# scottschroeder/shirley-raytracing-rs

Measured on AMD Instinct MI355X. Metric: Msamples/sec (whole node) on book-1 random_scene 1200x800 @ 500spp; 1/2/4/8 GPU, higher is better.
Workload: dtype f64

## Files before the change

### shirley-raytracing-rs_amd/csrc/rt/rt_api.cpp

```cpp
#include <algorithm>
#include <cmath>
#include <cstdlib>
#include <cstring>
#include <limits>
#include <string>
#include <vector>

#include "adaptive.h"
#include "plan.h"
#include "rt_ctx.h"

using namespace rt;

namespace rt {

int ensure(rt_ctx* c, DevBuf& b, size_t bytes) {
  if (b.bytes >= bytes && b.p) return RT_OK;
  if (c) HIP_TRY(c, hipSetDevice(c->device));
  if (b.p) {
    (void)hipFree(b.p);
    b.p = nullptr;
    b.bytes = 0;
  }
  if (bytes == 0) return RT_OK;
// ... 362 lines not shown
      w.q_window = (uint32_t)std::max(1, atoi(e) / kWave) * (uint32_t)kWave;
    KBlock& kb = c->host_blocks[k];
    kb.cam = kp.cam;
    kb.scene = kp.scene;
    kb.work = w;
    kb.partial = kp.partial;
    kb.unit_counter = kp.unit_counter;
    kb.counters = kp.counters;
    kb.ground = c->place.hop_kind == 2 ? static_cast<const DGround*>(c->ground.p) : nullptr;
    void* kdev = static_cast<KBlock*>(c->kcam.p) + k;
    HIP_TRY(c, hipMemcpyAsync(kdev, &kb, sizeof(KBlock), hipMemcpyHostToDevice, s));
    kp.kconst = (uint64_t)(uintptr_t)kdev;
    HIP_TRY(c, hipMemsetAsync(c->unit_counter.p, 0, std::max<size_t>(64, (size_t)nseg * sizeof(uint32_t)), s));
    HIP_TRY(c, hipEventRecord(c->pass_ev[2 * k], s));
    if (engine == RT_ENGINE_WAVEFRONT) {
      st = run_wavefront(c, kp, timing, s);
      if (st) return st;
    } else if (engine == RT_ENGINE_SPLIT) {
      kp.split_refill = c->split_refill;
      KParams ks = kp;
      ks.scene.n_lds_mats = ks.scene.n_lds_texs = 0;
      HIP_TRY(c, launch_split(ks, c->split_nt, c->cu_count, s));
    } else {
      HIP_TRY(c, launch_trace(kp, (int)nseg, c->place.mk_threads, c->place.hop_kind, s));
    }
    HIP_TRY(c, hipEventRecord(c->pass_ev[2 * k + 1], s));
    if (k == passes - 1) HIP_TRY(c, hipEventRecord(c->ev[1], s));
    if (step)
      HIP_TRY(c, launch_fold_stats(kp.partial, w.n_chunks, step->n_list, step->list_dev, L.tiles_x, cam->image_width,
                                   cam->image_height, step->batches_before + c1, step->batch, step->noise_floor,
                                   out_dev, step->moments_dev, step->err_dev, s));
    else
      HIP_TRY(c, launch_reduce(kp.partial, w.n_chunks, L.n_tiles_rank, L.tiles_x, ty0, p->tile_rank, p->tile_world,
                               cam->image_width, row0, row1, packed, k > 0 ? 1 : 0, out_dev, s));
    c->last_passes = k + 1;
  }
  HIP_TRY(c, hipEventRecord(c->ev[2], s));
  c->have_timing = true;
  return RT_OK;
}

}

extern "C" {

const char* rt_version(void) { return "shirley-rt 0.2 (gfx950, f64 wavefront + persistent megakernel)"; }

// ... 89 lines not shown
  if ((st = up(c->prim_light, cs.prim_light))) return st;
  if ((st = ensure(c, c->shutter0, 2 * sizeof(double)))) return st;
  HIP_TRY(c, hipMemset(c->shutter0.p, 0, 2 * sizeof(double)));

  DScene& S = c->scene;
  S.nodes = static_cast<const DNode*>(c->nodes.p);
  S.nodes4 = c->nodes4.p;
  S.prims = static_cast<const DPrim*>(c->prims.p);
  S.mats = static_cast<const DMat*>(c->mats.p);
  S.texs = static_cast<const DTex*>(c->texs.p);
  S.perlin = static_cast<const DPerlin*>(c->perlin.p);
  S.exts = cs.exts.empty() ? nullptr : static_cast<const DExt*>(c->exts.p);
  S.time0 = S.time1 = 0.0;
  S.shutter = static_cast<const double*>(c->shutter0.p);
  S.n_nodes = (int32_t)cs.nodes.size();
  S.n_nodes4 = cs.stats.n_nodes4;
  S.n_prims = cs.stats.n_objects;
  place_scene(P, S);
  S.sky = d->sky;
  for (int k = 0; k < 3; ++k) S.sky_color[k] = d->sky_color[k];
  c->place = P;

  int bpc = 0;
  HIP_TRY(c, trace_occupancy(S, P.mk_threads, P.hop_kind, &bpc));
  if (bpc < 1) return fail(c, RT_E_UNSUPPORTED, "trace kernel does not fit on a CU (LDS %lld B)", P.stack_bytes);
  c->blocks_per_cu = bpc;
  DScene W = S;
  W.n_lds_mats = W.n_lds_texs = 0;
  W.n_lds_nodes = P.wf_n_lds_nodes;
  int wbpc = 0;
  HIP_TRY(c, wf_prepare(W, &wbpc));
  if (wbpc < 1) return fail(c, RT_E_UNSUPPORTED, "wavefront extend kernel does not fit on a CU");
  c->wf_scene = W;
  c->wf_blocks_per_cu = wbpc;
  c->wf_wide = false;
  if (P.wf_extend4) {
    int b4 = 0;
    HIP_TRY(c, wf_prepare4(S, &b4));
    if (b4 >= 1) {
      c->wf_wide = true;
      c->wf4_blocks_per_cu = b4;
      c->wf_scene = S;
      c->wf_scene.n_lds_mats = c->wf_scene.n_lds_texs = 0;
    }
  }
  c->split_nt = 0;
  if (P.split_nt) {
// ... 418 lines not shown
```

### shirley-raytracing-rs_amd/csrc/rt/rt_device.h

```cpp
#pragma once

#ifdef RT_PORTABLE_LIBM
#include "portable_libm.h"
#define RT_SIN pl_sin
#define RT_LOG pl_log
#define RT_ACOS pl_acos
#define RT_ATAN2 pl_atan2
#define RT_POW5_LIBM(x) pl_pow5(x)
#else
#define RT_SIN sin
#define RT_LOG log
#define RT_ACOS acos
#define RT_ATAN2 atan2
#define RT_POW5_LIBM(x) pow(x, 5.0)
#endif
#include <hip/hip_runtime.h>

#include "../../../include/shirley_rt.h"
#include "rt_layout.h"

namespace rt {


struct v3 {
// ... 812 lines not shown
    } else if (h0) {
      next = c0;
    } else if (h1) {
      next = c1;
    } else {
      next = -1;
      while (sp > 0) {
        --sp;
        if ((double)stk_t[sp * STRIDE] <= t_best) {
          next = stk_node[sp * STRIDE];
          break;
        }
      }
      if (next < 0) break;
    }
    node = next;
  }
  resolve_ties<EXT>(S, o, d, t_min, t_best, best, face_best, rk, seed);
  return best;
}

#ifdef RT_PHASE_TIMING
#define g_trav_lane_steps trav_lane_steps_ref
static __device__ unsigned long long g_phase_ctr[64];
static __device__ unsigned long long g_visit_hist[64], g_wave_visit_hist[64];

__device__ __forceinline__ void ph_count(int i) {
  const unsigned long long act = __ballot(1);
  if ((int)__lane_id() == __builtin_ctzll(act)) {
    atomicAdd(&g_phase_ctr[2 * i], (unsigned long long)__popcll(act));
    atomicAdd(&g_phase_ctr[2 * i + 1], 1ull);
  }
}
#ifndef RT_PHASE_NO_EVENTS
#define PH_COUNT(i) ph_count(i)
#else
#define PH_COUNT(i)
#endif
#else
#define PH_COUNT(i)
#endif
#ifdef RT_PHASE_TIMING
#define RT_STAT(x) x
#define RT_STAT_ARG(x) , x
#else
#define RT_STAT(x)
#define RT_STAT_ARG(x)
// ... 407 lines not shown
__device__ __noinline__ RootHit traverse4_root_ool(const DNode4F* lds_nodes, const DPrim* lds_prims, const DPrim* prims_v,
                                                   int root4, unsigned key_mask, float origin_limit, v3 o, v3 d, Rng rk,
                                                   uint64_t seed_v) {
  DScene S{};
  S.prims = uniform_ptr(prims_v);
  S.root4 = __builtin_amdgcn_readfirstlane(root4);
  S.key_mask = (unsigned)__builtin_amdgcn_readfirstlane((int)key_mask);
  S.origin_limit = __int_as_float(__builtin_amdgcn_readfirstlane(__float_as_int(origin_limit)));
  RootHit r{0, -1, -1, __builtin_inf()};
  unsigned visits = 0, ptests = 0;
  r.ok = traverse4_root<MODE>(S, lds_nodes, lds_prims, o, d, 0.001, r.t, r.best, r.face, rk, uniform64(seed_v), visits,
                              ptests)
             ? 1
             : 0;
  return r;
}
#endif

__device__ __forceinline__ bool box_inward(int face, v3 d) {
  const double da = face < 2 ? d.z : (face < 4 ? d.x : d.y);
  return (face & 1) ? da > 0.0 : da < 0.0;
}
typedef __attribute__((address_space(4))) const DGround GGround;
__device__ __forceinline__ bool ground_hop(const DScene& S, const DPrim* lds_prims, const DMat* mats, GGround* g, v3 o, v3 d,
                                           double t_min, double& t_best, int& best, int& face_best, bool& guarded) {
  bool div_ok;
  const v3 inv = inv_dir(d, div_ok);
  const RaySigns ns = ray_signs(inv);
  t_best = __builtin_inf();
  best = -1;
  face_best = -1;
  const int n = g->n, n_box = g->n_box;
#pragma unroll 1
  for (int i = 0; i < n; ++i) {
    const int leaf = g->prim[i];
    const DPrim& pr = lds_prims[leaf];
    double te, t;
    if (i < n_box) {
      double tx;
      if (!slab_s(pr.p, o, inv, ns, t_min, t_best, te, tx)) {
        mark_tie<false>(best, near_entry(te, t_best));
        continue;
      }
      const int f = div_ok ? box_t1f(pr.p, o, d, inv, ns, t_min, t_best, te, tx, t) : box_t(pr.p, o, d, t_min, t_best, t, inv, div_ok);
      if (f >= 0 && tie_takes<false>(S, leaf, best, t, t_best, o, inv, ns, t_min)) { t_best = t; best = leaf; face_best = f; }
    } else {
      double b[6];
      leaf_box(pr, b);
      if (!slab_s(b, o, inv, ns, t_min, t_best, te)) continue;
      if (rect_t<0, 2>(pr.p, o, d, t_min, t_best, t, inv, div_ok) && tie_takes<false>(S, leaf, best, t, t_best, o, inv, ns, t_min)) {
        t_best = t; best = leaf; face_best = -1;
      }
    }
  }
  guarded = false;
  if (best < 0 || (best & kTieBit) || face_best < 4 || !(t_best > t_min)) return false;
  const DPrim& pb = lds_prims[best];
  const double ay = fabs(d.y);
  bool ok = mats[pb.material].kind == RT_MAT_DIELECTRIC && o.y >= g->y_lo && o.y <= g->y_hi && ay >= g->dy_min &&
            ay <= 0x1p300 && d.x * d.x + d.z * d.z <= g->ratio2 * (d.y * d.y);
  if (ok && (face_best == 4 ? pb.p[4] : pb.p[1]) == g->y_top) {
    const int nx = g->nx;
    const int ix = ground_cell(o.x + t_best * d.x, g->x0, nx), iz = ground_cell(o.z + t_best * d.z, g->z0, g->nz);
    if (ix >= 0 && iz >= 0) {
      typedef __attribute__((address_space(1))) const uint32_t GBits;
      const unsigned c = (unsigned)iz * (unsigned)nx + (unsigned)ix;
      GBits* bits = (GBits*)(uintptr_t)((uint64_t)(uintptr_t)g + sizeof(DGround));
      guarded = (bits[c >> 5] >> (c & 31u)) & 1u;
      ok = !guarded;
    }
  }
  return ok;
}

struct Trav4 {
  v3 inv;
  Recip ra;
  bool ra_ok;
  double t_best;
  float tmaxf;
  int best, face, node, sp, steps;
  unsigned top;
  RaySigns ns;
  RayF rf;
};

template <bool EXT>
__device__ __forceinline__ void trav4_begin(Trav4& T, const DScene& S, v3 o, v3 d, double t_max) {
  bool inv_ok;
  T.inv = inv_dir(d, inv_ok);
  T.ns = ray_signs(T.inv);
  T.rf = ray_f<typename Node4Sel<EXT>::T>(S, o, T.inv);
  T.ra = recip(len2(d));
  T.ra_ok = inv_ok && T.ra.b >= 0x1p-300 && T.ra.b <= 0x1p300 && T.rf.fast;
  T.t_best = t_max;
// ... 767 lines not shown
```

### shirley-raytracing-rs_amd/csrc/rt/rt_layout.h

```cpp
#pragma once

#include <stddef.h>
#include <stdint.h>

#include "plan.h"

namespace rt {

constexpr int kTile = 8;
constexpr int kTilePixels = kTile * kTile;
constexpr int kTraceThreads = 256;
constexpr int kTraceThreadsWide = 1024;
#ifndef RT_EXT_WIDE_THREADS
#define RT_EXT_WIDE_THREADS 768
#endif
constexpr int kTraceThreadsWide3 = RT_EXT_WIDE_THREADS;
constexpr int kHitThreads = 256;
constexpr int kExtendThreads = 256;
constexpr int kWave = 64;
constexpr int kLdsBytes = 160 * 1024;

constexpr int32_t kEmptyChild = 0x7fffffff;
struct alignas(16) DNode {
  double box[2][6];
// ... 114 lines not shown
  int32_t sky;
  double sky_color[3];
  const DExt* exts;
  double time0, time1;
  const double* shutter;
  int32_t n_lds_mats;
  int32_t n_lds_texs;
};

constexpr int kGroundMaxPrims = 4;
constexpr double kGroundCellsPerUnit = 32.0;
constexpr double kGroundCell = 1.0 / kGroundCellsPerUnit;
constexpr double kGroundGuard = 1.0 / 32.0;
constexpr long long kGroundMaxCells = 128LL * 1024 * 8;
struct alignas(16) DGround {
  double y_lo, y_hi;
  double y_top;
  double dy_min;
  double ratio2;
  double x0, z0;
  int32_t nx, nz;
  int32_t n, n_box;
  int32_t prim[kGroundMaxPrims];
  int32_t pad[2];
};
static_assert(sizeof(DGround) == 96, "DGround layout");
#ifdef __HIPCC__
#define RT_HOST_DEVICE __host__ __device__
#else
#define RT_HOST_DEVICE
#endif
RT_HOST_DEVICE inline int ground_cell(double v, double v0, int n) {
  const double q = (v - v0) * kGroundCellsPerUnit;
  return (q >= 0.0 && q < (double)n) ? (int)q : -1;
}

struct DCamera {
  int32_t width, height;
  int32_t has_lens;
  int32_t pad;
  double lens_radius;
  double origin[3], u[3], v[3];
  double horizontal[3], vertical[3], lower_left[3];
  double wd, hd, inv_w, inv_h;
};

struct UDiv {
// ... 117 lines not shown
```

### shirley-raytracing-rs_amd/csrc/rt/scene_compile.cpp

```cpp
#include "scene_compile.h"

#include <algorithm>
#include <cmath>
#include <cstdarg>
#include <cstdio>
#include <cstdlib>
#include <cstring>
#include <limits>

namespace rt {

namespace {
int fail(std::string* err, int code, const char* fmt, ...) {
  char buf[512];
  va_list ap;
  va_start(ap, fmt);
  vsnprintf(buf, sizeof buf, fmt, ap);
  va_end(ap);
  if (err) *err = buf;
  return code;
}
}

SceneTuning tuning_from_env() {
  SceneTuning t;
  if (const char* e = getenv("SHIRLEY_COLLAPSE_DP")) t.collapse_dp = atoi(e) != 0;
  if (const char* e = getenv("SHIRLEY_LDS_NODES")) {
    t.has_lds_nodes = true;
    t.lds_nodes = atoll(e);
  }
  t.no_wide = getenv("SHIRLEY_NO_WIDE") != nullptr;
  t.no_lds_prims = getenv("SHIRLEY_NO_LDS_PRIMS") != nullptr;
  t.no_lds_mats = getenv("SHIRLEY_NO_LDS_MATS") != nullptr;
  t.no_lds_perlin = getenv("SHIRLEY_NO_LDS_PERLIN") != nullptr;
  t.no_hop = getenv("SHIRLEY_NO_HOP") != nullptr;
  if (const char* e = getenv("SHIRLEY_HOP")) t.hop_root = std::strcmp(e, "root") == 0;
  if (const char* e = getenv("SHIRLEY_SAH_BOXW")) t.sah_box_weight = atof(e);
  t.sah_binned = getenv("SHIRLEY_SAH_BINNED") != nullptr;
  t.wf_extend2 = getenv("SHIRLEY_WF_EXTEND2") != nullptr;
  if (const char* e = getenv("SHIRLEY_SPLIT_NT")) t.split_nt = atoi(e);
  if (const char* e = getenv("SHIRLEY_SPLIT_REFILL")) t.split_refill = std::max(1, atoi(e));
  return t;
}

bool is_extended(const rt_object& o) {
  return o.geometry == RT_GEOM_MOVING_SPHERE || o.medium != 0 || o.transform != 0;
}
void rotate_y_cs(const rt_object& o, double& cs, double& sn) {
  const double rad = o.rotate_y_deg * 3.14159265358979323846 / 180.0;
  cs = std::cos(rad);
  sn = std::sin(rad);
}
bool texture_uses_uv(const rt_scene_desc* d, int32_t ti) {
  if (ti < 0 || ti >= d->n_textures) return false;
  const rt_texture& t = d->textures[ti];
  if (t.kind == RT_TEX_IMAGE) return true;
  if (t.kind == RT_TEX_CHECKER) return texture_uses_uv(d, t.odd) || texture_uses_uv(d, t.even);
  return false;
}
// ... 499 lines not shown
    if (!(lo_y >= top) || !(std::fabs(p[0]) <= big && std::fabs(p[1]) <= big && std::fabs(p[2]) <= big)) return false;
    const double dx = std::max(std::fabs(p[0] - ex0), std::fabs(p[0] - ex1));
    const double dy = std::max(std::fabs(p[1] - low), std::fabs(p[1] - top));
    const double dz = std::max(std::fabs(p[2] - ez0), std::fabs(p[2] - ez1));
    dist = std::max(dist, std::sqrt(dx * dx + dy * dy + dz * dz));
    if (lo_y - top < kGroundGuard / 2) guarded.push_back(&q);
  }
  const double ratio = 0x1p10, tol = 0x1p-40 * std::max(1.0, std::max(std::fabs(top), std::fabs(low)));
  const double reach = ((top - low) + 2.0 * tol) * (ratio + 1.0);
  const double l2 = (dist + reach) * (dist + reach) + reach * reach + r_max * r_max;
  const double m = 0x1p-38 * l2;
  const double eta = std::isfinite(r_min) ? m / (2.0 * r_min) : 0.0;
  if (!(eta <= 0x1p-16 && m <= 0x1p-13)) return false;
  const double gap = 4.0 * eta + 4.0 * tol;
  for (double y : planes)
    if (y != top && !(y <= top - gap)) return false;

  DGround g;
  std::memset(&g, 0, sizeof g);
  g.y_lo = low - tol;
  g.y_hi = top + tol;
  g.y_top = top;
  g.dy_min = std::max((2.0 * eta + 4.0 * tol) / 0.001, 0x1p-100);
  g.ratio2 = ratio * ratio;
  g.n = (int32_t)n_g;
  g.n_box = (int32_t)boxes.size();
  for (size_t i = 0; i < boxes.size(); ++i) g.prim[i] = boxes[i];
  for (size_t i = 0; i < rects.size(); ++i) g.prim[boxes.size() + i] = rects[i];
  size_t words = 0;
  if (!guarded.empty()) {
    double cx0 = guarded[0]->p[0], cx1 = cx0, cz0 = guarded[0]->p[2], cz1 = cz0;
    for (const DPrim* q : guarded) {
      cx0 = std::min(cx0, q->p[0]), cx1 = std::max(cx1, q->p[0]);
      cz0 = std::min(cz0, q->p[2]), cz1 = std::max(cz1, q->p[2]);
    }
    g.x0 = std::floor(cx0 * kGroundCellsPerUnit - 2.0) * kGroundCell;
    g.z0 = std::floor(cz0 * kGroundCellsPerUnit - 2.0) * kGroundCell;
    const double nx = std::ceil((cx1 - g.x0) * kGroundCellsPerUnit + 2.0), nz = std::ceil((cz1 - g.z0) * kGroundCellsPerUnit + 2.0);
    if (!(nx * nz <= (double)kGroundMaxCells)) return false;
    g.nx = (int32_t)nx;
    g.nz = (int32_t)nz;
    words = ((size_t)g.nx * (size_t)g.nz + 31) / 32;
  }
  out.assign(sizeof(DGround) / 4 + words, 0u);
  std::memcpy(out.data(), &g, sizeof g);
  uint32_t* bits = out.data() + sizeof(DGround) / 4;
// ... 52 lines not shown
    return fail(err, RT_E_UNSUPPORTED, "BVH too deep for the LDS traversal stack (depth %d)", depth);
  P.wide = wide_lds(0, 0, 0, 0) <= (size_t)kLdsBytes && (placement == 0 || placement == RT_BVH_NODES_LDS) &&
           !tune.no_wide;
  P.mk_threads = P.wide ? wide_threads : kTraceThreads;
  P.n_lds_nodes = lds_nodes_for(kHitThreads * 8LL * P.stack_depth);
  P.n_lds_nodes4 = P.wide ? n_nodes4 : lds_count(stack4_bytes, n4_bytes, nodes4.size());
  const bool prims_lds = P.wide && wide_lds(d->n_objects, 0, n_mats, n_texs) <= (size_t)kLdsBytes &&
                         !tune.no_lds_prims && !tune.no_lds_mats;
  P.n_lds_prims = prims_lds ? d->n_objects : 0;
  const bool perlin_lds = prims_lds && d->n_perlin > 0 &&
                          wide_lds(d->n_objects, d->n_perlin, n_mats, n_texs) <= (size_t)kLdsBytes &&
                          !tune.no_lds_perlin;
  P.n_lds_perlin = perlin_lds ? d->n_perlin : 0;
  P.n_lds_mats = prims_lds ? n_mats : 0;
  P.n_lds_texs = prims_lds ? n_texs : 0;
  bool coat = false;
  for (int i = 0; i < d->n_objects && !coat; ++i) {
    const rt_object& o = d->objects[i];
    coat = o.geometry == RT_GEOM_RECT_BOX && d->materials[o.material].kind == RT_MAT_DIELECTRIC;
  }
  P.hop_pass = coat && !ext && prims_lds && !tune.no_hop;
  P.hop_kind = !P.hop_pass ? 0 : (!tune.hop_root && ground_stack(cs.prims, d->n_objects, cs.ground)) ? 2 : 1;
  if (P.hop_kind != 2) cs.ground.clear();

  const long long wf_stack = (long long)wf_extend_lds(0, P.stack_depth);
  if (wf_stack > kLdsBytes)
    return fail(err, RT_E_UNSUPPORTED, "BVH too deep for the LDS traversal stack (depth %d)", depth);
  P.wf_n_lds_nodes = lds_nodes_for(wf_stack);
  P.wf_extend4 = P.wide && P.n_lds_prims > 0 && !tune.wf_extend2;
  if (P.wide && !ext && P.n_lds_prims == d->n_objects) {
    P.split_nt = tune.split_nt;
    P.split_refill = tune.split_refill;
  }

  cs.stats.n_objects = d->n_objects;
  cs.stats.n_nodes = (int32_t)tree.nodes.size();
  int32_t leaves = 0;
  for (const auto& n : tree.nodes) leaves += n.leaf >= 0;
  cs.stats.n_leaves = leaves;
  cs.stats.depth = depth;
  cs.stats.n_nodes4 = n_nodes4;
  cs.stats.wide_block = P.wide ? 1 : 0;
  cs.stats.origin_limit = P.origin_limit;
  cs.stats.hop_pass = P.hop_pass ? 1 : 0;
  cs.stats.hop_kind = P.hop_kind;
  cs.stats.device_bytes = (int64_t)(cs.nodes.size() * sizeof(DNode) + cs.prims.size() * sizeof(DPrim) +
// ... 343 lines not shown
```

### shirley-raytracing-rs_amd/csrc/rt/scene_compile.h

```cpp
#pragma once

#include <stdint.h>

#include <string>
#include <utility>
#include <vector>

#include "../../../include/shirley_rt.h"
#include "bvh_build.h"
#include "rt_layout.h"

namespace rt {

constexpr int32_t kPlacementMask = RT_BVH_NODES_GLOBAL | RT_BVH_NODES_HALF_LDS | RT_BVH_NODES_LDS;

struct SceneTuning {
  int collapse_dp = -1;
  bool has_lds_nodes = false;
  long long lds_nodes = 0;
  bool no_wide = false;
  bool no_lds_prims = false;
  bool no_lds_mats = false;
  bool no_lds_perlin = false;
  bool no_hop = false;
  bool hop_root = false;
  double sah_box_weight = 4.0;
  bool sah_binned = false;
  bool wf_extend2 = false;
  int split_nt = 8;
  int split_refill = 0;
};
SceneTuning tuning_from_env();

struct ScenePlacement {
  bool wide = false;
  int mk_threads = kTraceThreads;
  bool collapse_dp = false;
  int32_t n_lds_nodes = 0, n_lds_nodes4 = 0, n_lds_prims = 0, n_lds_perlin = 0, n_lds_mats = 0, n_lds_texs = 0;
  int32_t stack_depth = 0, stack_depth4 = 0, root4 = 0;
  long long stack_bytes = 0;
  uint32_t key_mask = 0;
  float origin_limit = 0.f;
  int32_t wf_n_lds_nodes = 0;
  bool wf_extend4 = false;
  int split_nt = 0;
  int split_refill = 0;
  bool hop_pass = false;
  int hop_kind = 0;
};

inline void place_scene(const ScenePlacement& P, DScene& S) {
  S.stack_depth = P.stack_depth;
  S.stack_depth4 = P.stack_depth4;
  S.root4 = P.root4;
  S.key_mask = P.key_mask;
  S.origin_limit = P.origin_limit;
  S.n_lds_nodes = P.n_lds_nodes;
  S.n_lds_nodes4 = P.n_lds_nodes4;
  S.n_lds_prims = P.n_lds_prims;
  S.n_lds_perlin = P.n_lds_perlin;
  S.n_lds_mats = P.n_lds_mats;
  S.n_lds_texs = P.n_lds_texs;
}

struct LightList {
  std::vector<rt_light> lights;
  std::vector<DLight> dev;
  int32_t n_unlisted = 0;
};
LightList list_lights(const rt_scene_desc* d);

constexpr double kLightPickWeighted = 0.875;
// ... 53 lines not shown
```

### shirley-raytracing-rs_amd/csrc/rt/trace.hip

```cpp
#include "adaptive.h"
#include "rt_device.h"
#include "pass_frame.h"
#include "rt_launch.h"

#include <algorithm>
#include <vector>

namespace rt {

__device__ __forceinline__ unsigned long long lanemask_lt() {
  unsigned lane = __lane_id();
  return (lane == 0) ? 0ull : ((~0ull) >> (64 - lane));
}

__host__ __device__ inline size_t lds_bytes(int n_lds_nodes, int stack_depth, int stride) {
  return (size_t)n_lds_nodes * sizeof(DNode) + (size_t)stack_depth * stride * 8;
}

#ifndef RT_KSCENE
#define RT_KSCENE 1
#endif
#ifndef RT_NARROW_WAVES
#define RT_NARROW_WAVES 4
#endif
constexpr int kNarrowWaves = RT_NARROW_WAVES;
#ifndef RT_NARROW_WAVES_EXT
#define RT_NARROW_WAVES_EXT 3
#endif

#ifndef RT_HOP_MIN_LANES
#define RT_HOP_MIN_LANES 40
#endif
#ifndef RT_HOP2_INSIDE
#define RT_HOP2_INSIDE 1
#endif
#ifndef RT_HOP2_MIN_LANES_A
#define RT_HOP2_MIN_LANES_A 24
#endif
#ifndef RT_HOP2_MIN_LANES_B
#define RT_HOP2_MIN_LANES_B 16
#endif
template <int THREADS, int MODE, bool EXT, bool LIST = false, int HOP = 0>
__global__ __launch_bounds__(THREADS, THREADS >= kTraceThreadsWide3 ? 1 : (EXT ? RT_NARROW_WAVES_EXT : kNarrowWaves))
void trace_kernel(KParams P) {
  extern __shared__ unsigned char lds_raw[];
  const int tid = threadIdx.x;
  typedef typename Node4Sel<EXT>::T N4;
  N4* lds_nodes = reinterpret_cast<N4*>(lds_raw);
  DPrim* lds_prims = reinterpret_cast<DPrim*>(lds_raw + (size_t)P.scene.n_lds_nodes4 * sizeof(N4));
  const DPerlin* lds_perlin = (MODE == kSceneLds && P.scene.n_lds_perlin > 0)
                                  ? reinterpret_cast<const DPerlin*>(lds_prims + P.scene.n_lds_prims)
                                  : nullptr;
  unsigned char* stk_base = lds_raw + (size_t)P.scene.n_lds_nodes4 * sizeof(N4) +
                            (MODE == kSceneLds ? (size_t)P.scene.n_lds_prims * sizeof(DPrim) +
                                                     (size_t)P.scene.n_lds_perlin * sizeof(DPerlin) +
                                                     (size_t)P.scene.n_lds_mats * sizeof(DMat) +
                                                     (size_t)P.scene.n_lds_texs * sizeof(DTex)
                                               : 0);
  unsigned* stk = reinterpret_cast<unsigned*>(stk_base) + tid;
  stage_nodes4<MODE>(P.scene, lds_nodes, lds_prims);
  const DMat* mats = P.scene.mats;
  const DTex* texs = P.scene.texs;
  if constexpr (MODE == kSceneLds) {
// ... 38 lines not shown
  do {              \
  } while (0)
#endif
#ifdef RT_TIMELINE
  const unsigned wave_gid = blockIdx.x * (THREADS / kWave) + tid / kWave;
  bool ph_exh_seen = false;
  if (lane == 0 && wave_gid < (unsigned)kTimelineWaves) g_wave_t0[wave_gid] = __builtin_amdgcn_s_memrealtime();
#endif
  for (;;) {
#if defined(RT_PHASE_TIMING) && !defined(RT_PHASE_NO_EVENTS)
    const unsigned long long ph_before = ph_lane_steps;
#endif
    const DScene& S = P.scene;
    bool hit = false, need_pn = false, need_r = false;
    int prim = -1, face = -1, leaf = -1, mat = 0, ptab = 0, mk = -1;
    double t_best = __builtin_inf(), psc = 0.0;
    Hit h;
    h.point = V(0.0, 0.0, 0.0);
    h.normal = h.point;
    h.t = h.u = h.v = 0.0;
    h.front_face = false;
    PH_COUNT(6);
    n_seg += __popcll(__ballot(active));
    if (active) {
      prim = traverse4<THREADS, MODE, EXT>(S, lds_nodes, lds_prims, o, d, 0.001, t_best, face, stk, rng, seed, visits,
                                      ptests RT_STAT_ARG(ph_lane_steps));
#ifdef RT_PHASE_TIMING
    }
    PH_STAMP(kPhTrav);
    {
#endif
      if (prim >= 0) {
        PH_COUNT(15);
        hit = true;
        const DPrim pr = (MODE == kSceneLds) ? lds_prims[prim] : S.prims[prim];
        hit_record<false, EXT>(S, pr, face, o, d, t_best, rng, seed, h);
        mat = pr.material;
        mk = mats[mat].kind;
        need_r = mk == RT_MAT_LAMBERTIAN || mk == RT_MAT_METAL || mk == RT_MAT_FAIRY_LIGHT || mk == RT_MAT_ISOTROPIC;
        if (mk == RT_MAT_LAMBERTIAN || mk == RT_MAT_FAIRY_LIGHT || mk == RT_MAT_DIFFUSE_LIGHT || mk == RT_MAT_ISOTROPIC) {
          leaf = resolve_texture_t(texs, mats[mat].tex, h.point);
          const DTex& tx = texs[leaf];
          if (tx.kind == RT_TEX_PERLIN) {
            need_pn = true;
            ptab = tx.table;
            psc = tx.scale;
          }
        }
      }
    }
    PH_STAMP(kPhRecord);
    const bool ends = active && (!hit || mk == RT_MAT_DIFFUSE_LIGHT);
    const bool free_lane = !active || ends;
    bool publish = false;
    uint32_t pub_index = 0;
    if (free_lane && has_unit && rng.sample + 1u >= (uint32_t)s_end) {
      publish = true;
      pub_index = part_index;
      has_unit = false;
    }
    bool need = free_lane && !has_unit;
    unsigned long long mask = __ballot(need);
    if (mask != 0ull && !exhausted) {
      unsigned long long k = __popcll(mask);
      unsigned long long rank = __popcll(mask & lanemask_lt());
      unsigned long long avail = w_end - w_next;
      unsigned long long idx;
      unsigned win = kSegmentWindow;
      if (avail >= k) {
        idx = w_next + rank;
        w_next += k;
      } else {
        KBlk* kb = kblock(P.kconst);
        unsigned long long nb = kb->work.n_units;
        if (kb->work.n_segs != 0u) {
// ... 63 lines not shown
        if (px < kc->width && py < kc->height) {
          PH_COUNT(10);
          has_unit = true;
          const int s0 = kw->sample_base + chunk * kw->chunk;
          s_end = min(kw->samples, s0 + kw->chunk);
          rng.sample = (uint32_t)s0 - 1u;
          rng.pixel = (uint32_t)py * (uint32_t)kc->width + (uint32_t)px;
          pxy = (uint32_t)px | ((uint32_t)py << 16);
          part_index = (uint32_t)chunk * ((uint32_t)kw->n_tiles_rank * (uint32_t)kTilePixels) +
                       lt * (uint32_t)kTilePixels + (uint32_t)lp;
        }
      }
    }
    const bool regen = free_lane && has_unit;
    n_samp += __popcll(__ballot(regen));
    if (regen) {
      rng.sample += 1u;
      rng.draw = 0;
    }
    PH_STAMP(kPhRegen);
    const double pn = lds_perlin ? marble_coop((LdsPerlin*)lds_perlin, need_pn, ptab, psc, h.point)
                                 : marble_coop(S.perlin, need_pn, ptab, psc, h.point);
    PH_STAMP(kPhMarble);
    const bool scat = active && !ends;
    const int dk = regen ? kDrawCam
                         : (scat && need_r) ? kDrawSphere : (scat && mk == RT_MAT_DIELECTRIC) ? kDrawDiel : kDrawNone;
    double jx = 0.0, jy = 0.0;
    const v3 rs = draws_coop(rng, seed, dk, C.has_lens != 0, pxy, jx, jy);
    const v3 un = unit_fast(!active ? V(1.0, 1.0, 1.0) : (scat && need_r && mk != RT_MAT_METAL) ? rs : d);
    PH_STAMP(kPhDraws);
    if (regen) {
      PH_COUNT(11);
      camera_ray_drawn(kblock(P.kconst)->cam, jx, jy, rs, o, d);
    }
    PH_STAMP(kPhCamera);
    if (active) {
      bool alive, has_emit = false;
      v3 mul = V(1.0, 1.0, 1.0), emit = V(0.0, 0.0, 0.0);
      if (hit) {
        const DMat& m = mats[mat];
        alive = shade_factor(S, texs, m, leaf, pn, rs, un, rng, o, d, h, prim, face, mul, emit, has_emit);
      } else {
        PH_COUNT(20);
#if RT_KSCENE
        emit = sky_unit(kblock(P.kconst)->scene, un);
#else
        emit = sky_unit(S, un);
#endif
        has_emit = true;
        alive = false;
      }
      if (has_emit) em = em + hmul(att, emit);
      att = hmul(att, mul);
      if (alive) alive = --depth_left > 0;
      if (!alive) {
        sum = sum + em;
        active = false;
      }
    }
// ... 32 lines not shown
          f_hop = rh.face;
#else
          serve = traverse4_root<MODE>(S, lds_nodes, lds_prims, o, d, 0.001, t_hop, p_hop, f_hop, rng, seed, visits, ptests);
#endif
          if (serve) serve = mats[lds_prims[p_hop].material].kind == RT_MAT_DIELECTRIC;
        }
        n_seg += __popcll(__ballot(serve));
        if (serve) {
          PH_COUNT(27);
          const DPrim pr = lds_prims[p_hop];
          Hit hh;
          hit_record<false, false>(S, pr, f_hop, o, d, t_hop, rng, seed, hh);
          const v3 ru = draw_diel(rng, seed);
          const v3 ud = unit_fast(d);
          shade_dielectric(mats[pr.material], ru, ud, rng, o, d, hh);
          if (--depth_left <= 0) {
            sum = sum + em;
            active = false;
          }
        }
      }
      PH_STAMP(kPhTail);
    }
    if constexpr (HOP == 2) {
      static_assert(MODE == kSceneLds && !EXT, "the hop pass is built for the scene-in-LDS reference-scene instances");
      bool cand = active && !regen && hit;
      if (cand) cand = lds_prims[prim].kind != kPrimSphere;
#if RT_HOP2_INSIDE
      if (cand && face >= 0) cand = box_inward(face, d);
#endif
#pragma unroll 1
      for (int run = 0; run < 2; ++run) {
        if (__popcll(__ballot(cand)) < (run ? RT_HOP2_MIN_LANES_B : RT_HOP2_MIN_LANES_A)) break;
        bool serve = false;
        double t_hop = __builtin_inf();
        int p_hop = -1, f_hop = -1;
        if (cand) {
          if (run) PH_COUNT(28); else PH_COUNT(26);
          bool guarded;
          serve = ground_hop(S, lds_prims, mats, (GGround*)kblock(P.kconst)->ground, o, d, 0.001, t_hop, p_hop, f_hop, guarded);
          if (guarded) PH_COUNT(30);
        }
        n_seg += __popcll(__ballot(serve));
        if (serve) {
          if (run) PH_COUNT(29); else PH_COUNT(27);
          const DPrim pr = lds_prims[p_hop];
          Hit hh;
          hit_record<false, false>(S, pr, f_hop, o, d, t_hop, rng, seed, hh);
          const v3 ru = draw_diel(rng, seed);
          const v3 ud = unit_fast(d);
          shade_dielectric(mats[pr.material], ru, ud, rng, o, d, hh);
          if (--depth_left <= 0) {
            sum = sum + em;
            active = false;
          }
        }
        cand = serve && active;
#if RT_HOP2_INSIDE
        if (cand) cand = box_inward(f_hop, d);
#endif
      }
      PH_STAMP(kPhTail);
    }
#ifdef RT_TIMELINE
    if (exhausted && !ph_exh_seen) {
      ph_exh_seen = true;
      if (lane == 0 && wave_gid < (unsigned)kTimelineWaves) g_wave_tx[wave_gid] = __builtin_amdgcn_s_memrealtime();
    }
#endif
    if (exhausted && !__any(active || has_unit)) break;
#if defined(RT_PHASE_TIMING) && !defined(RT_PHASE_NO_EVENTS)
    {
      unsigned dl = (unsigned)(ph_lane_steps - ph_before);
      if (dl > 0) atomicAdd(&g_visit_hist[min(dl, 63u)], 1ull);
// ... 378 lines not shown
template <int THREADS, int MODE>
static void launch_trace1(const KParams& p, int blocks, size_t lds, hipStream_t stream) {
  if (p.scene.exts)
    launch_trace2<THREADS, MODE, true>(p, blocks, lds, stream);
  else
    launch_trace2<THREADS, MODE, false>(p, blocks, lds, stream);
}

static hipError_t hit_prepare(const DScene& S) {
  const int lds = (int)hit_lds_bytes(S.n_lds_nodes, S.stack_depth);
  switch (node_mode(S)) {
    case kNodesLds: return hipFuncSetAttribute((const void*)hit_kernel<kNodesLds>, hipFuncAttributeMaxDynamicSharedMemorySize, lds);
    case kNodesGlobal: return hipFuncSetAttribute((const void*)hit_kernel<kNodesGlobal>, hipFuncAttributeMaxDynamicSharedMemorySize, lds);
    default: return hipFuncSetAttribute((const void*)hit_kernel<kNodesMixed>, hipFuncAttributeMaxDynamicSharedMemorySize, lds);
  }
}

hipError_t trace_occupancy(const DScene& S, int threads, int hop, int* blocks_per_cu) {
  hipError_t e = hit_prepare(S);
  if (e != hipSuccess) return e;
  if (hop && !(threads == kTraceThreadsWide && !S.exts && S.n_lds_prims > 0)) return hipErrorInvalidValue;
  if (threads == kTraceThreadsWide && !S.exts) {
    if (node_mode4(S) != kNodesLds) return hipErrorInvalidValue;
    if (hop == 2) return occupancy_impl1<kTraceThreadsWide, kSceneLds, false, 2>(S, blocks_per_cu);
    if (hop) return occupancy_impl1<kTraceThreadsWide, kSceneLds, false, 1>(S, blocks_per_cu);
    if (S.n_lds_prims > 0) return occupancy_impl1<kTraceThreadsWide, kSceneLds, false>(S, blocks_per_cu);
    return occupancy_impl1<kTraceThreadsWide, kNodesLds, false>(S, blocks_per_cu);
  }
  if (threads == kTraceThreadsWide3) {
    if (node_mode4(S) != kNodesLds || !S.exts) return hipErrorInvalidValue;
    if (S.n_lds_prims > 0) return occupancy_impl1<kTraceThreadsWide3, kSceneLds, true>(S, blocks_per_cu);
    return occupancy_impl1<kTraceThreadsWide3, kNodesLds, true>(S, blocks_per_cu);
  }
  switch (node_mode4(S)) {
    case kNodesLds: return occupancy_impl<kTraceThreads, kNodesLds>(S, blocks_per_cu);
    case kNodesGlobal: return occupancy_impl<kTraceThreads, kNodesGlobal>(S, blocks_per_cu);
    default: return occupancy_impl<kTraceThreads, kNodesMixed>(S, blocks_per_cu);
  }
}

hipError_t launch_trace(const KParams& p, int blocks, int threads, int hop, hipStream_t stream) {
  const size_t lds = trace_lds_bytes(p.scene.n_lds_nodes4, node4_bytes(p.scene.exts != nullptr), p.scene.n_lds_prims, p.scene.n_lds_perlin, p.scene.stack_depth4, threads,
                                     p.scene.n_lds_mats, p.scene.n_lds_texs);
  if (hop && !(threads == kTraceThreadsWide && !p.scene.exts && p.scene.n_lds_prims > 0)) return hipErrorInvalidValue;
  if (threads == kTraceThreadsWide && !p.scene.exts) {
    if (hop == 2)
      launch_trace2<kTraceThreadsWide, kSceneLds, false, 2>(p, blocks, lds, stream);
    else if (hop)
      launch_trace2<kTraceThreadsWide, kSceneLds, false, 1>(p, blocks, lds, stream);
    else if (p.scene.n_lds_prims > 0)
      launch_trace2<kTraceThreadsWide, kSceneLds, false>(p, blocks, lds, stream);
    else
      launch_trace2<kTraceThreadsWide, kNodesLds, false>(p, blocks, lds, stream);
    return hipGetLastError();
  }
  if (threads == kTraceThreadsWide3) {
    if (!p.scene.exts) return hipErrorInvalidValue;
    if (p.scene.n_lds_prims > 0)
      launch_trace2<kTraceThreadsWide3, kSceneLds, true>(p, blocks, lds, stream);
    else
      launch_trace2<kTraceThreadsWide3, kNodesLds, true>(p, blocks, lds, stream);
    return hipGetLastError();
  }
  switch (node_mode4(p.scene)) {
    case kNodesLds: launch_trace1<kTraceThreads, kNodesLds>(p, blocks, lds, stream); break;
    case kNodesGlobal: launch_trace1<kTraceThreads, kNodesGlobal>(p, blocks, lds, stream); break;
    default: launch_trace1<kTraceThreads, kNodesMixed>(p, blocks, lds, stream);
  }
  return hipGetLastError();
// ... 100 lines not shown
          }
        }
      auto pct = [](std::vector<double> v, double q) {
        if (v.empty()) return 0.0;
        std::sort(v.begin(), v.end());
        return v[std::min(v.size() - 1, (size_t)(q * (double)(v.size() - 1)))];
      };
      fprintf(stderr, "[phase-timeline] waves %zu; exit us p0 %.1f p50 %.1f p90 %.1f p99 %.1f p99.9 %.1f max %.1f; "
              "pool exhausted seen at us p0 %.1f p50 %.1f; exhausted->exit us p50 %.1f p90 %.1f p99 %.1f max %.1f\n",
              ends.size(), pct(ends, 0), pct(ends, 0.5), pct(ends, 0.9), pct(ends, 0.99), pct(ends, 0.999),
              pct(ends, 1), pct(firstx, 0), pct(firstx, 0.5), pct(tails, 0.5), pct(tails, 0.9), pct(tails, 0.99),
              pct(tails, 1));
      std::fill(t0, t0 + kTimelineWaves, 0ull);
      (void)hipMemcpyToSymbol(HIP_SYMBOL(g_wave_t0), t0, sizeof t0);
      (void)hipMemcpyToSymbol(HIP_SYMBOL(g_wave_tx), t0, sizeof t0);
      (void)hipMemcpyToSymbol(HIP_SYMBOL(g_wave_t1), t0, sizeof t0);
    }
  }
}
#endif

#ifdef RT_PHASE_TIMING
void phase_counters_dump() {
  unsigned long long h[64];
  if (hipMemcpyFromSymbol(h, HIP_SYMBOL(g_phase_ctr), sizeof h) != hipSuccess) return;
  static const char* names[] = {"visit", "visit_with_leaves", "sphere_iter", "sphere_slab_pass", "rect_iter",
                                "pop_iter", "segment_iter", "box_iter", "marble_round", "draws_coop_round",
                                "unit_fetch", "camera_ray", "philox_A", "philox_B", "marble_sin", "hit_record",
                                "checker_level", "dielectric", "metal", "lambertian", "sky", "diffuse_light",
                                "reflectance", "traverse4", "publish", "tie_resolve", "hop_candidate", "hop_served",
                                "hop2_candidate", "hop2_served", "hop_guarded"};
  for (int i = 0; i < 31; ++i)
    if (h[2 * i + 1])
      fprintf(stderr, "[phase-ev] %-18s lanes %.4g waves %.4g lanes/wave %.2f\n", names[i], (double)h[2 * i],
              (double)h[2 * i + 1], (double)h[2 * i] / (double)h[2 * i + 1]);
  unsigned long long lh[64], wh[64];
  if (hipMemcpyFromSymbol(lh, HIP_SYMBOL(g_visit_hist), sizeof lh) == hipSuccess &&
      hipMemcpyFromSymbol(wh, HIP_SYMBOL(g_wave_visit_hist), sizeof wh) == hipSuccess) {
    fprintf(stderr, "[phase-hist] visits: lanes / waves (slowest lane)\n");
    for (int i = 1; i < 64; ++i)
      if (lh[i] || wh[i]) fprintf(stderr, "[phase-hist] %2d %.6g %.6g\n", i, (double)lh[i], (double)wh[i]);
  }
  unsigned long long z[64] = {};
  (void)hipMemcpyToSymbol(HIP_SYMBOL(g_phase_ctr), z, sizeof z);
  (void)hipMemcpyToSymbol(HIP_SYMBOL(g_visit_hist), z, sizeof z);
  (void)hipMemcpyToSymbol(HIP_SYMBOL(g_wave_visit_hist), z, sizeof z);
}
#endif

hipError_t launch_tonemap(const double* accum, int width, int height, double inv, uint8_t* rgb8, hipStream_t stream) {
  const long long n = (long long)width * height * 3;
  const int blocks = (int)((n + 255) / 256);
  if (blocks == 0) return hipSuccess;
  hipLaunchKernelGGL(tonemap_kernel, dim3(blocks), dim3(256), 0, stream, accum, width, height, inv, rgb8);
  return hipGetLastError();
}

hipError_t launch_unpack(const double* gathered, int world, int max_tiles, int n_tiles_total, int tiles_x, int width,
                         int height, double* out, hipStream_t stream) {
  long long n = (long long)world * max_tiles * kTilePixels;
  int blocks = (int)((n + 255) / 256);
  if (blocks == 0) return hipSuccess;
  hipLaunchKernelGGL(unpack_kernel, dim3(blocks), dim3(256), 0, stream, gathered, world, max_tiles, n_tiles_total,
                     tiles_x, width, height, out);
  return hipGetLastError();
}

}
```

Measured before the change: 3044.

## Add downward ground-hop pass serving dielectric ground hits before full traversal

Adds a new trace instance (hop 3) that, after traversal hits a dielectric ground primitive, shades the refraction inline and tries a cheap ground-only intersection (ground_hop_t<DOWN>) instead of a full BVH traversal. It repeats up to three rounds while enough lanes in the wave qualify, and uses a 'waiting' state to defer lanes that still need a full traversal. A host-side check enables it only when a non-dielectric ground primitive lies below the new y_down threshold, and the DGround padding is replaced by that y_down field. This aims to cut BVH traversals for rays passing through the glass ground layer, at the cost of a larger kernel, more divergence and register pressure. It also extends the phase-timing event counters.

```diff
diff --git a/shirley-raytracing-rs_amd/csrc/rt/rt_api.cpp b/shirley-raytracing-rs_amd/csrc/rt/rt_api.cpp
--- a/shirley-raytracing-rs_amd/csrc/rt/rt_api.cpp
+++ b/shirley-raytracing-rs_amd/csrc/rt/rt_api.cpp
@@ -408,7 +408,7 @@
       ks.scene.n_lds_mats = ks.scene.n_lds_texs = 0;
       HIP_TRY(c, launch_split(ks, c->split_nt, c->cu_count, s));
     } else {
-      HIP_TRY(c, launch_trace(kp, (int)nseg, c->place.mk_threads, c->place.hop_kind, s));
+      HIP_TRY(c, launch_trace(kp, (int)nseg, c->place.mk_threads, hop_instance(c->place), s));
     }
     HIP_TRY(c, hipEventRecord(c->pass_ev[2 * k + 1], s));
     if (k == passes - 1) HIP_TRY(c, hipEventRecord(c->ev[1], s));
@@ -544,7 +544,7 @@
   c->place = P;
 
   int bpc = 0;
-  HIP_TRY(c, trace_occupancy(S, P.mk_threads, P.hop_kind, &bpc));
+  HIP_TRY(c, trace_occupancy(S, P.mk_threads, hop_instance(P), &bpc));
   if (bpc < 1) return fail(c, RT_E_UNSUPPORTED, "trace kernel does not fit on a CU (LDS %lld B)", P.stack_bytes);
   c->blocks_per_cu = bpc;
   DScene W = S;
diff --git a/shirley-raytracing-rs_amd/csrc/rt/rt_device.h b/shirley-raytracing-rs_amd/csrc/rt/rt_device.h
--- a/shirley-raytracing-rs_amd/csrc/rt/rt_device.h
+++ b/shirley-raytracing-rs_amd/csrc/rt/rt_device.h
@@ -858,7 +858,8 @@
 
 #ifdef RT_PHASE_TIMING
 #define g_trav_lane_steps trav_lane_steps_ref
-static __device__ unsigned long long g_phase_ctr[64];
+constexpr int kPhaseEvents = 48;
+static __device__ unsigned long long g_phase_ctr[2 * kPhaseEvents];
 static __device__ unsigned long long g_visit_hist[64], g_wave_visit_hist[64];
 
 __device__ __forceinline__ void ph_count(int i) {
@@ -1312,8 +1313,10 @@
   return (face & 1) ? da > 0.0 : da < 0.0;
 }
 typedef __attribute__((address_space(4))) const DGround GGround;
-__device__ __forceinline__ bool ground_hop(const DScene& S, const DPrim* lds_prims, const DMat* mats, GGround* g, v3 o, v3 d,
-                                           double t_min, double& t_best, int& best, int& face_best, bool& guarded) {
+constexpr int kHopRefused = 0, kHopServed = 1, kHopFound = 2;
+template <bool DOWN>
+__device__ __forceinline__ int ground_hop_t(const DScene& S, const DPrim* lds_prims, const DMat* mats, GGround* g, v3 o, v3 d,
+                                            double t_min, double& t_best, int& best, int& face_best, bool& guarded) {
   bool div_ok;
   const v3 inv = inv_dir(d, div_ok);
   const RaySigns ns = ray_signs(inv);
@@ -1344,11 +1347,21 @@
     }
   }
   guarded = false;
-  if (best < 0 || (best & kTieBit) || face_best < 4 || !(t_best > t_min)) return false;
+  if (best < 0 || (best & kTieBit) || (DOWN ? face_best >= 0 && face_best < 4 : face_best < 4) || !(t_best > t_min))
+    return kHopRefused;
   const DPrim& pb = lds_prims[best];
   const double ay = fabs(d.y);
-  bool ok = mats[pb.material].kind == RT_MAT_DIELECTRIC && o.y >= g->y_lo && o.y <= g->y_hi && ay >= g->dy_min &&
-            ay <= 0x1p300 && d.x * d.x + d.z * d.z <= g->ratio2 * (d.y * d.y);
+  const bool diel = mats[pb.material].kind == RT_MAT_DIELECTRIC;
+  const bool slab_ok = o.y >= g->y_lo && o.y <= g->y_hi && ay >= g->dy_min && ay <= 0x1p300 &&
+                       d.x * d.x + d.z * d.z <= g->ratio2 * (d.y * d.y);
+  if constexpr (DOWN) {
+    if (!diel) {
+      const double y = face_best < 0 ? pb.p[4] + 0.0001 : (face_best == 4 ? pb.p[4] : pb.p[1]);
+      return (slab_ok && y <= g->y_down) ? kHopFound : kHopRefused;
+    }
+    if (face_best < 4) return kHopRefused;
+  }
+  bool ok = diel && slab_ok;
   if (ok && (face_best == 4 ? pb.p[4] : pb.p[1]) == g->y_top) {
     const int nx = g->nx;
     const int ix = ground_cell(o.x + t_best * d.x, g->x0, nx), iz = ground_cell(o.z + t_best * d.z, g->z0, g->nz);
@@ -1360,7 +1373,11 @@
       ok = !guarded;
     }
   }
-  return ok;
+  return ok ? kHopServed : kHopRefused;
+}
+__device__ __forceinline__ bool ground_hop(const DScene& S, const DPrim* lds_prims, const DMat* mats, GGround* g, v3 o, v3 d,
+                                           double t_min, double& t_best, int& best, int& face_best, bool& guarded) {
+  return ground_hop_t<false>(S, lds_prims, mats, g, o, d, t_min, t_best, best, face_best, guarded) != kHopRefused;
 }
 
 struct Trav4 {
diff --git a/shirley-raytracing-rs_amd/csrc/rt/rt_layout.h b/shirley-raytracing-rs_amd/csrc/rt/rt_layout.h
--- a/shirley-raytracing-rs_amd/csrc/rt/rt_layout.h
+++ b/shirley-raytracing-rs_amd/csrc/rt/rt_layout.h
@@ -160,7 +160,7 @@
   int32_t nx, nz;
   int32_t n, n_box;
   int32_t prim[kGroundMaxPrims];
-  int32_t pad[2];
+  double y_down;
 };
 static_assert(sizeof(DGround) == 96, "DGround layout");
 #ifdef __HIPCC__
diff --git a/shirley-raytracing-rs_amd/csrc/rt/scene_compile.cpp b/shirley-raytracing-rs_amd/csrc/rt/scene_compile.cpp
--- a/shirley-raytracing-rs_amd/csrc/rt/scene_compile.cpp
+++ b/shirley-raytracing-rs_amd/csrc/rt/scene_compile.cpp
@@ -34,7 +34,10 @@
   t.no_lds_mats = getenv("SHIRLEY_NO_LDS_MATS") != nullptr;
   t.no_lds_perlin = getenv("SHIRLEY_NO_LDS_PERLIN") != nullptr;
   t.no_hop = getenv("SHIRLEY_NO_HOP") != nullptr;
-  if (const char* e = getenv("SHIRLEY_HOP")) t.hop_root = std::strcmp(e, "root") == 0;
+  if (const char* e = getenv("SHIRLEY_HOP")) {
+    t.hop_root = std::strcmp(e, "root") == 0;
+    t.hop_up = std::strcmp(e, "up") == 0;
+  }
   if (const char* e = getenv("SHIRLEY_SAH_BOXW")) t.sah_box_weight = atof(e);
   t.sah_binned = getenv("SHIRLEY_SAH_BINNED") != nullptr;
   t.wf_extend2 = getenv("SHIRLEY_WF_EXTEND2") != nullptr;
@@ -580,6 +583,7 @@
   g.y_hi = top + tol;
   g.y_top = top;
   g.dy_min = std::max((2.0 * eta + 4.0 * tol) / 0.001, 0x1p-100);
+  g.y_down = top - gap;
   g.ratio2 = ratio * ratio;
   g.n = (int32_t)n_g;
   g.n_box = (int32_t)boxes.size();
@@ -678,6 +682,16 @@
   P.hop_pass = coat && !ext && prims_lds && !tune.no_hop;
   P.hop_kind = !P.hop_pass ? 0 : (!tune.hop_root && ground_stack(cs.prims, d->n_objects, cs.ground)) ? 2 : 1;
   if (P.hop_kind != 2) cs.ground.clear();
+  P.hop_down = false;
+  if (P.hop_kind == 2 && !tune.hop_up) {
+    DGround g;
+    std::memcpy(&g, cs.ground.data(), sizeof g);
+    for (int i = 0; i < g.n && !P.hop_down; ++i) {
+      const DPrim& q = cs.prims[g.prim[i]];
+      if (cs.mats[q.material].kind == RT_MAT_DIELECTRIC) continue;
+      P.hop_down = i < g.n_box ? (q.p[1] <= g.y_down || q.p[4] <= g.y_down) : q.p[4] + 0.0001 <= g.y_down;
+    }
+  }
 
   const long long wf_stack = (long long)wf_extend_lds(0, P.stack_depth);
   if (wf_stack > kLdsBytes)
diff --git a/shirley-raytracing-rs_amd/csrc/rt/scene_compile.h b/shirley-raytracing-rs_amd/csrc/rt/scene_compile.h
--- a/shirley-raytracing-rs_amd/csrc/rt/scene_compile.h
+++ b/shirley-raytracing-rs_amd/csrc/rt/scene_compile.h
@@ -24,6 +24,7 @@
   bool no_lds_perlin = false;
   bool no_hop = false;
   bool hop_root = false;
+  bool hop_up = false;
   double sah_box_weight = 4.0;
   bool sah_binned = false;
   bool wf_extend2 = false;
@@ -47,7 +48,10 @@
   int split_refill = 0;
   bool hop_pass = false;
   int hop_kind = 0;
+  bool hop_down = false;
 };
+
+inline int hop_instance(const ScenePlacement& P) { return P.hop_kind == 2 && P.hop_down ? 3 : P.hop_kind; }
 
 inline void place_scene(const ScenePlacement& P, DScene& S) {
   S.stack_depth = P.stack_depth;
diff --git a/shirley-raytracing-rs_amd/csrc/rt/trace.hip b/shirley-raytracing-rs_amd/csrc/rt/trace.hip
--- a/shirley-raytracing-rs_amd/csrc/rt/trace.hip
+++ b/shirley-raytracing-rs_amd/csrc/rt/trace.hip
@@ -39,6 +39,39 @@
 #endif
 #ifndef RT_HOP2_MIN_LANES_B
 #define RT_HOP2_MIN_LANES_B 16
+#endif
+#ifndef RT_HOPD_MIN_LANES_A
+#define RT_HOPD_MIN_LANES_A 32
+#endif
+#ifndef RT_HOPD_MIN_LANES_B
+#define RT_HOPD_MIN_LANES_B 16
+#endif
+#ifndef RT_HOPD_MIN_LANES_C
+#define RT_HOPD_MIN_LANES_C 16
+#endif
+#ifndef RT_HOP3_MIN_LANES_A
+#define RT_HOP3_MIN_LANES_A RT_HOP2_MIN_LANES_A
+#endif
+#ifndef RT_HOP3_MIN_LANES_B
+#define RT_HOP3_MIN_LANES_B RT_HOP2_MIN_LANES_B
+#endif
+#ifdef RT_HOP_SERVE_SHARED
+struct ServeOut {
+  v3 o, d;
+  uint32_t draw, c2, c3;
+};
+__device__ __noinline__ ServeOut hop_serve_ool(const DPrim* lds_prims, const DMat* mats, int prim, int face, v3 o, v3 d,
+                                               double t, Rng rng, uint64_t seed_v) {
+  DScene S{};
+  const uint64_t seed = uniform64(seed_v);
+  const DPrim pr = lds_prims[prim];
+  Hit hh;
+  hit_record<false, false>(S, pr, face, o, d, t, rng, seed, hh);
+  const v3 ru = draw_diel(rng, seed);
+  const v3 ud = unit_fast(d);
+  shade_dielectric(mats[pr.material], ru, ud, rng, o, d, hh);
+  return ServeOut{o, d, rng.draw, rng.c2, rng.c3};
+}
 #endif
 template <int THREADS, int MODE, bool EXT, bool LIST = false, int HOP = 0>
 __global__ __launch_bounds__(THREADS, THREADS >= kTraceThreadsWide3 ? 1 : (EXT ? RT_NARROW_WAVES_EXT : kNarrowWaves))
@@ -123,9 +156,71 @@
     h.front_face = false;
     PH_COUNT(6);
     n_seg += __popcll(__ballot(active));
+    bool waiting = false;
+    if constexpr (HOP == 3) {
+      static_assert(MODE == kSceneLds && !EXT, "the hop pass is built for the scene-in-LDS reference-scene instances");
+      if (active)
+        prim = traverse4<THREADS, MODE, EXT>(S, lds_nodes, lds_prims, o, d, 0.001, t_best, face, stk, rng, seed, visits,
+                                             ptests RT_STAT_ARG(ph_lane_steps));
+      PH_STAMP(kPhTrav);
+      GGround* g = (GGround*)kblock(P.kconst)->ground;
+      bool pend = false;
+      if (active && prim >= 0 && mats[lds_prims[prim].material].kind == RT_MAT_DIELECTRIC)
+        for (int i = 0; i < g->n; ++i) pend = pend || g->prim[i] == prim;
+#if defined(RT_PHASE_TIMING) && !defined(RT_PHASE_NO_EVENTS)
+      if (pend) PH_COUNT(31);
+#endif
+#pragma unroll 1
+      for (int run = 0; run < 3; ++run) {
+        if (__popcll(__ballot(pend)) <
+            (run == 0 ? RT_HOPD_MIN_LANES_A : (run == 1 ? RT_HOPD_MIN_LANES_B : RT_HOPD_MIN_LANES_C)))
+          break;
+        int kind = kHopRefused;
+        if (pend) {
+          PH_COUNT(36 + 4 * run);
+          pend = false;
+#ifdef RT_HOP_SERVE_SHARED
+          const ServeOut so = hop_serve_ool(lds_prims, mats, prim, face, o, d, t_best, rng, seed);
+          o = so.o, d = so.d, rng.draw = so.draw, rng.c2 = so.c2, rng.c3 = so.c3;
+#else
+          const DPrim pr = lds_prims[prim];
+          Hit hh;
+          hit_record<false, false>(S, pr, face, o, d, t_best, rng, seed, hh);
+          const v3 ru = draw_diel(rng, seed);
+          const v3 ud = unit_fast(d);
+          shade_dielectric(mats[pr.material], ru, ud, rng, o, d, hh);
+#endif
+          if (--depth_left <= 0) {
+            sum = sum + em;
+            active = false;
+          }
+          const bool inward = face < 0 || d.y < 0.0 || box_inward(face, d);
+          prim = -1;
+          waiting = active;
+          if (active && inward) {
+            double t_hop;
+            int p_hop, f_hop;
+            bool guarded;
+            kind = ground_hop_t<true>(S, lds_prims, mats, g, o, d, 0.001, t_hop, p_hop, f_hop, guarded);
+            if (kind != kHopRefused) {
+              prim = p_hop;
+              face = f_hop;
+              t_best = t_hop;
+              waiting = false;
+              pend = kind == kHopServed;
+              if (pend) PH_COUNT(37 + 4 * run); else PH_COUNT(38 + 4 * run);
+            }
+          }
+          if (waiting) PH_COUNT(39 + 4 * run);
+        }
+        n_seg += __popcll(__ballot(kind != kHopRefused));
+      }
+      PH_STAMP(kPhTrav);
+    }
     if (active) {
-      prim = traverse4<THREADS, MODE, EXT>(S, lds_nodes, lds_prims, o, d, 0.001, t_best, face, stk, rng, seed, visits,
-                                      ptests RT_STAT_ARG(ph_lane_steps));
+      if constexpr (HOP != 3)
+        prim = traverse4<THREADS, MODE, EXT>(S, lds_nodes, lds_prims, o, d, 0.001, t_best, face, stk, rng, seed, visits,
+                                        ptests RT_STAT_ARG(ph_lane_steps));
 #ifdef RT_PHASE_TIMING
     }
     PH_STAMP(kPhTrav);
@@ -151,7 +246,24 @@
       }
     }
     PH_STAMP(kPhRecord);
-    const bool ends = active && (!hit || mk == RT_MAT_DIFFUSE_LIGHT);
+#if defined(RT_PHASE_TIMING) && !defined(RT_PHASE_NO_EVENTS)
+    if constexpr (HOP == 2) {
+      bool dg = false;
+      if (hit && mk == RT_MAT_DIELECTRIC) {
+        GGround* g = (GGround*)kblock(P.kconst)->ground;
+        for (int i = 0; i < g->n; ++i) dg = dg || g->prim[i] == prim;
+      }
+      const int n_dg = __popcll(__ballot(dg));
+      if (dg) {
+        PH_COUNT(31);
+        if (n_dg >= 8) PH_COUNT(32);
+        if (n_dg >= 16) PH_COUNT(33);
+        if (n_dg >= 24) PH_COUNT(34);
+        if (n_dg >= 32) PH_COUNT(35);
+      }
+    }
+#endif
+    const bool ends = active && !waiting && (!hit || mk == RT_MAT_DIFFUSE_LIGHT);
     const bool free_lane = !active || ends;
     bool publish = false;
     uint32_t pub_index = 0;
@@ -261,7 +373,7 @@
     const double pn = lds_perlin ? marble_coop((LdsPerlin*)lds_perlin, need_pn, ptab, psc, h.point)
                                  : marble_coop(S.perlin, need_pn, ptab, psc, h.point);
     PH_STAMP(kPhMarble);
-    const bool scat = active && !ends;
+    const bool scat = active && !ends && !waiting;
     const int dk = regen ? kDrawCam
                          : (scat && need_r) ? kDrawSphere : (scat && mk == RT_MAT_DIELECTRIC) ? kDrawDiel : kDrawNone;
     double jx = 0.0, jy = 0.0;
@@ -273,7 +385,7 @@
       camera_ray_drawn(kblock(P.kconst)->cam, jx, jy, rs, o, d);
     }
     PH_STAMP(kPhCamera);
-    if (active) {
+    if (active && !waiting) {
       bool alive, has_emit = false;
       v3 mul = V(1.0, 1.0, 1.0), emit = V(0.0, 0.0, 0.0);
       if (hit) {
@@ -352,7 +464,7 @@
       }
       PH_STAMP(kPhTail);
     }
-    if constexpr (HOP == 2) {
+    if constexpr (HOP == 2 || HOP == 3) {
       static_assert(MODE == kSceneLds && !EXT, "the hop pass is built for the scene-in-LDS reference-scene instances");
       bool cand = active && !regen && hit;
       if (cand) cand = lds_prims[prim].kind != kPrimSphere;
@@ -361,7 +473,9 @@
 #endif
 #pragma unroll 1
       for (int run = 0; run < 2; ++run) {
-        if (__popcll(__ballot(cand)) < (run ? RT_HOP2_MIN_LANES_B : RT_HOP2_MIN_LANES_A)) break;
+        if (__popcll(__ballot(cand)) < (HOP == 3 ? (run ? RT_HOP3_MIN_LANES_B : RT_HOP3_MIN_LANES_A)
+                                                 : (run ? RT_HOP2_MIN_LANES_B : RT_HOP2_MIN_LANES_A)))
+          break;
         bool serve = false;
         double t_hop = __builtin_inf();
         int p_hop = -1, f_hop = -1;
@@ -374,12 +488,20 @@
         n_seg += __popcll(__ballot(serve));
         if (serve) {
           if (run) PH_COUNT(29); else PH_COUNT(27);
+#ifdef RT_HOP_SERVE_SHARED
+          if constexpr (HOP == 3) {
+            const ServeOut so = hop_serve_ool(lds_prims, mats, p_hop, f_hop, o, d, t_hop, rng, seed);
+            o = so.o, d = so.d, rng.draw = so.draw, rng.c2 = so.c2, rng.c3 = so.c3;
+          } else
+#endif
+          {
           const DPrim pr = lds_prims[p_hop];
           Hit hh;
           hit_record<false, false>(S, pr, f_hop, o, d, t_hop, rng, seed, hh);
           const v3 ru = draw_diel(rng, seed);
           const v3 ud = unit_fast(d);
           shade_dielectric(mats[pr.material], ru, ud, rng, o, d, hh);
+          }
           if (--depth_left <= 0) {
             sum = sum + em;
             active = false;
@@ -804,6 +926,7 @@
   if (hop && !(threads == kTraceThreadsWide && !S.exts && S.n_lds_prims > 0)) return hipErrorInvalidValue;
   if (threads == kTraceThreadsWide && !S.exts) {
     if (node_mode4(S) != kNodesLds) return hipErrorInvalidValue;
+    if (hop == 3) return occupancy_impl1<kTraceThreadsWide, kSceneLds, false, 3>(S, blocks_per_cu);
     if (hop == 2) return occupancy_impl1<kTraceThreadsWide, kSceneLds, false, 2>(S, blocks_per_cu);
     if (hop) return occupancy_impl1<kTraceThreadsWide, kSceneLds, false, 1>(S, blocks_per_cu);
     if (S.n_lds_prims > 0) return occupancy_impl1<kTraceThreadsWide, kSceneLds, false>(S, blocks_per_cu);
@@ -826,7 +949,9 @@
                                      p.scene.n_lds_mats, p.scene.n_lds_texs);
   if (hop && !(threads == kTraceThreadsWide && !p.scene.exts && p.scene.n_lds_prims > 0)) return hipErrorInvalidValue;
   if (threads == kTraceThreadsWide && !p.scene.exts) {
-    if (hop == 2)
+    if (hop == 3)
+      launch_trace2<kTraceThreadsWide, kSceneLds, false, 3>(p, blocks, lds, stream);
+    else if (hop == 2)
       launch_trace2<kTraceThreadsWide, kSceneLds, false, 2>(p, blocks, lds, stream);
     else if (hop)
       launch_trace2<kTraceThreadsWide, kSceneLds, false, 1>(p, blocks, lds, stream);
@@ -973,15 +1098,20 @@
 
 #ifdef RT_PHASE_TIMING
 void phase_counters_dump() {
-  unsigned long long h[64];
+  unsigned long long h[2 * kPhaseEvents];
   if (hipMemcpyFromSymbol(h, HIP_SYMBOL(g_phase_ctr), sizeof h) != hipSuccess) return;
   static const char* names[] = {"visit", "visit_with_leaves", "sphere_iter", "sphere_slab_pass", "rect_iter",
                                 "pop_iter", "segment_iter", "box_iter", "marble_round", "draws_coop_round",
                                 "unit_fetch", "camera_ray", "philox_A", "philox_B", "marble_sin", "hit_record",
                                 "checker_level", "dielectric", "metal", "lambertian", "sky", "diffuse_light",
                                 "reflectance", "traverse4", "publish", "tie_resolve", "hop_candidate", "hop_served",
-                                "hop2_candidate", "hop2_served", "hop_guarded"};
-  for (int i = 0; i < 31; ++i)
+                                "hop2_candidate", "hop2_served", "hop_guarded",
+                                "down_hit", "down_hit_ge8", "down_hit_ge16", "down_hit_ge24", "down_hit_ge32",
+                                "down1_try", "down1_served", "down1_found", "down1_wait",
+                                "down2_try", "down2_served", "down2_found", "down2_wait",
+                                "down3_try", "down3_served", "down3_found", "down3_wait"};
+  static_assert(sizeof names / sizeof names[0] <= kPhaseEvents, "event slots");
+  for (int i = 0; i < (int)(sizeof names / sizeof names[0]); ++i)
     if (h[2 * i + 1])
       fprintf(stderr, "[phase-ev] %-18s lanes %.4g waves %.4g lanes/wave %.2f\n", names[i], (double)h[2 * i],
               (double)h[2 * i + 1], (double)h[2 * i] / (double)h[2 * i + 1]);
@@ -992,10 +1122,10 @@
     for (int i = 1; i < 64; ++i)
       if (lh[i] || wh[i]) fprintf(stderr, "[phase-hist] %2d %.6g %.6g\n", i, (double)lh[i], (double)wh[i]);
   }
-  unsigned long long z[64] = {};
+  unsigned long long z[2 * kPhaseEvents] = {};
   (void)hipMemcpyToSymbol(HIP_SYMBOL(g_phase_ctr), z, sizeof z);
-  (void)hipMemcpyToSymbol(HIP_SYMBOL(g_visit_hist), z, sizeof z);
-  (void)hipMemcpyToSymbol(HIP_SYMBOL(g_wave_visit_hist), z, sizeof z);
+  (void)hipMemcpyToSymbol(HIP_SYMBOL(g_visit_hist), z, 64 * sizeof z[0]);
+  (void)hipMemcpyToSymbol(HIP_SYMBOL(g_wave_visit_hist), z, 64 * sizeof z[0]);
 }
 #endif
 
```

Measured after the change: 3134 (median of 6 runs). 2.9% higher.
